# albcab/mfm

Hardware: AMD Instinct MI355X
Metric: MFM train-steps/s x chains (phi-four d=256, 4096 chains per GPU) (higher is better)
Workload: dtype f32

## Files before the change

### include/mfm.h

```cpp
#ifndef MFM_H
#define MFM_H

#include <stddef.h>
#include <stdint.h>

#ifdef __cplusplus
extern "C" {
#endif

typedef struct mfm_ctx mfm_ctx;

enum { MFM_OK = 0, MFM_EINVAL = -1, MFM_EUNSUPPORTED = -2, MFM_ETOOLARGE = -3, MFM_EHIP = -4, MFM_ENOTARGET = -5 };

enum { MFM_PHI4 = 0, MFM_GMM = 1, MFM_LGCP = 2 };
enum { MFM_FLOW_RWMH = 0, MFM_FLOW_IMH = 1 };
enum { MFM_FAMILY_AUTO = 0, MFM_FAMILY_TILE = 1, MFM_FAMILY_WIDE = 2 };
enum { MFM_ACT_RELU = 0, MFM_ACT_TANH = 1, MFM_ACT_ELU = 2, MFM_ACT_GELU = 3, MFM_ACT_SWISH = 4 };

#define MFM_MAX_DEPTH 3
typedef struct mfm_config {
  int32_t dim;
  int32_t fourier_dim;
  int32_t hidden_t[2];
  int32_t hidden_x[2];
// ... 76 lines not shown
int mfm_vf_apply(mfm_ctx* ctx, const float* d_x, const float* d_t, const float* d_tangent, int n,
                 float* d_v, float* d_jvp);
int mfm_ode_transform(mfm_ctx* ctx, int direction, int per_chain_keys, const uint32_t* d_keys, uint32_t key0,
                      uint32_t key1, const float* d_in, int n, float* d_out, float* d_ldj, int32_t* d_nsteps);
int mfm_flow_step(mfm_ctx* ctx, int mode, uint32_t key0, uint32_t key1, double beta,
                  float* d_pos, double* d_logp, float* d_grad,
                  float* d_acceptance_rate, uint8_t* d_is_accepted, float* d_proposed_position, int32_t* d_nsteps);

int mfm_train_iter(mfm_ctx* ctx, int64_t count, int mcmc_per_flow_steps, int flow_mode,
                   uint32_t gen_key0, uint32_t gen_key1, uint32_t train_key0, uint32_t train_key1,
                   double beta, double step_size, float* d_pos, double* d_logp, float* d_grad,
                   float* d_acceptance_rate, int32_t* d_nsteps, double* d_loss, float* d_grads, int apply_update);

int mfm_beta_update(mfm_ctx* ctx, double prev_beta, const double* d_logliks, int n, double alpha, double* h_beta_out);

int mfm_normal_rows(mfm_ctx* ctx, const uint32_t* d_keys, int n, float* d_out);

int mfm_cis_select(mfm_ctx* ctx, uint32_t key0, uint32_t key1, int n_is, const float* d_u0, const float* d_vol0,
                   const float* d_refs, const float* d_xs, const float* d_vols, const double* d_lps, float* d_pos,
                   double* d_logp, float* d_acc_prob, uint8_t* d_is_accepted, float* d_proposed, float* d_weight);

int mfm_stein_disc(mfm_ctx* ctx, const float* d_x, const float* d_grad, int n, double beta, double h_u_v[2]);
int mfm_max_mean_disc(mfm_ctx* ctx, const float* d_x, const float* d_y, int m, double* h_out);

#define MFM_AUTOCORR_LAG_BLOCK 32
#define MFM_AUTOCORR_TIME_BLOCK 256
int mfm_autocorr(mfm_ctx* ctx, const float* d_x, int64_t n, int64_t n_series, int32_t n_lags,
                 float* d_rho      ,
                 float* d_tau, float* d_ess ,
                 double* d_mean, double* d_var );

int mfm_noise_prefetch(mfm_ctx* ctx, int n_slots, const uint32_t* h_keys_gn, const uint32_t* h_keys_step);
int mfm_noise_drop(mfm_ctx* ctx);

int mfm_smc_delta(mfm_ctx* ctx, const double* d_loglik, int n, double target_ess, double max_delta, double* h_delta);
int mfm_smc_weights(mfm_ctx* ctx, const double* d_loglik, int n, double delta, double* d_weights, double* h_lognorm);
int mfm_smc_resample(mfm_ctx* ctx, uint32_t key0, uint32_t key1, const double* d_weights, int n, double* d_scratch,
                     int32_t* d_idx);
#define MFM_RESAMPLE_SYSTEMATIC 0
#define MFM_RESAMPLE_STRATIFIED 1
#define MFM_RESAMPLE_MULTINOMIAL 2
int mfm_smc_resample_scheme(mfm_ctx* ctx, int scheme, uint32_t key0, uint32_t key1, const double* d_weights, int n,
                            double* d_scratch, int32_t* d_idx);
int mfm_gather_rows(mfm_ctx* ctx, const float* d_src, const int32_t* d_idx, int n, int dim, float* d_dst);
int mfm_choice_logw(mfm_ctx* ctx, uint32_t key0, uint32_t key1, const double* d_logw, int n, int m, double* d_scratch,
                    int32_t* d_idx);
int mfm_acc_stats(mfm_ctx* ctx, const float* d_x, int n, double* d_out);

int mfm_get_counters(mfm_ctx* ctx, int64_t h_out[8]);
int mfm_reset_counters(mfm_ctx* ctx);

int mfm_debug_replay(mfm_ctx* ctx, int cap, const float* d_dt, const uint8_t* d_acc, float* d_ratio, float* d_dt_own,
                     double* d_diag);

int mfm_profile(mfm_ctx* ctx, int class_mask);
int mfm_profile_read(mfm_ctx* ctx, double ms_total[8], int64_t launches[8]);

int mfm_pack_index(int k, int n, int KB);
int mfm_pack_index_T(int k, int n, int NB);
int mfm_threefry2x32(uint32_t k0, uint32_t k1, uint32_t c0, uint32_t c1, uint32_t out[2]);

#ifdef __cplusplus
}
#endif
#endif
```

### mfm_amd/_lib.py

```python
import ctypes as C
import os

import numpy as np

from .build import LIB

PHI4, GMM, LGCP = 0, 1, 2
FLOW_RWMH, FLOW_IMH = 0, 1
FAMILY_AUTO, FAMILY_TILE, FAMILY_WIDE = 0, 1, 2
ACTIVATIONS = {"relu": 0, "tanh": 1, "elu": 2, "gelu": 3, "swish": 4}


class MfmError(RuntimeError):
    pass


class Config(C.Structure):
    _fields_ = [
        ("dim", C.c_int32), ("fourier_dim", C.c_int32),
        ("hidden_t", C.c_int32 * 2), ("hidden_x", C.c_int32 * 2), ("hidden_xt", C.c_int32 * 2),
        ("n_chain_local", C.c_int32), ("n_chain_total", C.c_int32), ("chain_offset", C.c_int32),
        ("grad_clip", C.c_float), ("sigma", C.c_float), ("cond_flow", C.c_int32), ("hutch", C.c_int32),
        ("rtol", C.c_double), ("atol", C.c_double), ("mxstep", C.c_int32), ("n_ts", C.c_int32),
        ("learning_rate", C.c_double), ("adam_b1", C.c_double), ("adam_b2", C.c_double), ("adam_eps", C.c_double),
# ... 31 lines not shown
    "mfm_mala_step_keys": (C.c_int, [_P, _P, C.c_double, C.c_double, C.c_int, _P, _P, _P, _P, _P, _P, _P]),
    "mfm_mala_run": (C.c_int, [_P, C.c_int, _U32, _U32, _P, C.c_double, C.c_double, C.c_int, C.c_int32, C.c_int32, _P, _P, _P, _P, _P, _P, _P, _P, _P, _P, _P]),
    "mfm_hmc_step": (C.c_int, [_P, _U32, _U32, C.c_double, C.c_double, C.c_int, _P, _P, _P, _P, _P]),
    "mfm_loglik": (C.c_int, [_P, _P, _P]),
    "mfm_smc_delta": (C.c_int, [_P, _P, C.c_int, C.c_double, C.c_double, C.POINTER(C.c_double)]),
    "mfm_smc_weights": (C.c_int, [_P, _P, C.c_int, C.c_double, _P, C.POINTER(C.c_double)]),
    "mfm_smc_resample": (C.c_int, [_P, _U32, _U32, _P, C.c_int, _P, _P]),
    "mfm_smc_resample_scheme": (C.c_int, [_P, C.c_int, _U32, _U32, _P, C.c_int, _P, _P]),
    "mfm_gather_rows": (C.c_int, [_P, _P, _P, C.c_int, C.c_int, _P]),
    "mfm_acc_stats": (C.c_int, [_P, _P, C.c_int, _P]),
    "mfm_choice_logw": (C.c_int, [_P, _U32, _U32, _P, C.c_int, C.c_int, _P, _P]),
    "mfm_fm_loss_grad": (C.c_int, [_P, _U32, _U32, _P, _P, _P]),
    "mfm_fm_loss": (C.c_int, [_P, _U32, _U32, _P, C.c_int, C.c_int, C.c_int, _P]),
    "mfm_adamw_step": (C.c_int, [_P, _P]),
    "mfm_comm_unique_id": (C.c_int, [_P]),
    "mfm_comm_init": (C.c_int, [_P, C.c_int, C.c_int, _P]),
    "mfm_comm_destroy": (C.c_int, [_P]),
    "mfm_comm_count": (C.c_int, [_P, _P]),
    "mfm_grad_allreduce_begin": (C.c_int, [_P, _P]),
    "mfm_opt_state": (C.c_int, [_P, C.POINTER(C.c_int32), C.POINTER(C.c_float)]),
    "mfm_vf_apply": (C.c_int, [_P, _P, _P, _P, C.c_int, _P, _P]),
    "mfm_ode_transform": (C.c_int, [_P, C.c_int, C.c_int, _P, _U32, _U32, _P, C.c_int, _P, _P, _P]),
    "mfm_flow_step": (C.c_int, [_P, C.c_int, _U32, _U32, C.c_double, _P, _P, _P, _P, _P, _P, _P]),
    "mfm_train_iter": (C.c_int, [_P, C.c_int64, C.c_int, C.c_int, _U32, _U32, _U32, _U32, C.c_double, C.c_double,
                                 _P, _P, _P, _P, _P, _P, _P, C.c_int]),
    "mfm_beta_update": (C.c_int, [_P, C.c_double, _P, C.c_int, C.c_double, C.POINTER(C.c_double)]),
    "mfm_normal_rows": (C.c_int, [_P, _P, C.c_int, _P]),
    "mfm_cis_select": (C.c_int, [_P, _U32, _U32, C.c_int, _P, _P, _P, _P, _P, _P, _P, _P, _P, _P, _P, _P]),
    "mfm_stein_disc": (C.c_int, [_P, _P, _P, C.c_int, C.c_double, C.POINTER(C.c_double)]),
    "mfm_max_mean_disc": (C.c_int, [_P, _P, _P, C.c_int, C.POINTER(C.c_double)]),
    "mfm_autocorr": (C.c_int, [_P, _P, C.c_int64, C.c_int64, C.c_int32, _P, _P, _P, _P, _P]),
    "mfm_noise_prefetch": (C.c_int, [_P, C.c_int, C.POINTER(_U32), C.POINTER(_U32)]),
    "mfm_noise_drop": (C.c_int, [_P]),
    "mfm_get_counters": (C.c_int, [_P, C.POINTER(C.c_int64)]),
    "mfm_reset_counters": (C.c_int, [_P]),
    "mfm_debug_replay": (C.c_int, [_P, C.c_int, _P, _P, _P, _P, _P]),
    "mfm_profile": (C.c_int, [_P, C.c_int]),
    "mfm_profile_read": (C.c_int, [_P, C.POINTER(C.c_double), C.POINTER(C.c_int64)]),
    "mfm_pack_index": (C.c_int, [C.c_int, C.c_int, C.c_int]),
    "mfm_pack_index_T": (C.c_int, [C.c_int, C.c_int, C.c_int]),
    "mfm_threefry2x32": (C.c_int, [_U32, _U32, _U32, _U32, C.POINTER(_U32)]),
}
EXPORTS = tuple(_SIGS)

_lib = None


def load():
    global _lib
    if _lib is None:
        if not os.path.exists(LIB):
            raise MfmError(f"{LIB} not found: build it with `python -m mfm_amd.build` (hipcc, gfx950)")
        import torch
        lib = C.CDLL(os.environ.get("MFM_LIB", LIB))
        for name, (res, args) in _SIGS.items():
            fn = getattr(lib, name)
            fn.restype, fn.argtypes = res, args
        _lib = lib
    return _lib


def _chk(rc):
    if rc != 0:
        raise MfmError(f"libmfm_hip error {rc}: {load().mfm_last_error().decode()}")


# ... 197 lines not shown
        self._p()
        _chk(self.lib.mfm_vf_apply(self.h, _ptr(x, F32), _ptr(t, F32), _ptr(tangent, F32), x.shape[0], _ptr(v, F32), _ptr(jvp, F32)))

    def ode_transform(self, direction, x, out, ldj, keys=None, key=(0, 0), nsteps=None):
        self._p()
        _chk(self.lib.mfm_ode_transform(self.h, direction, 0 if keys is None else 1, _ptr(keys, I32), int(key[0]), int(key[1]),
                                        _ptr(x, F32), x.shape[0], _ptr(out, F32), _ptr(ldj, F32), _ptr(nsteps, I32)))

    def flow_step(self, mode, key, beta, pos, logp, grad, acc=None, is_acc=None, proposed=None, nsteps=None):
        self._p()
        _chk(self.lib.mfm_flow_step(self.h, mode, int(key[0]), int(key[1]), float(beta), _ptr(pos, F32), _ptr(logp, F64), _ptr(grad, F32),
                                    _ptr(acc, F32), _ptr(is_acc, U8), _ptr(proposed, F32), _ptr(nsteps, I32)))

    def train_iter(self, count, mcmc_per_flow_steps, flow_mode, key_gen, key_train, beta, step_size, pos, logp, grad, loss, grads,
                   acc=None, nsteps=None, apply_update=True):
        self._p()
        _chk(self.lib.mfm_train_iter(self.h, int(count), int(mcmc_per_flow_steps), int(flow_mode), int(key_gen[0]), int(key_gen[1]),
                                     int(key_train[0]), int(key_train[1]), float(beta), float(step_size), _ptr(pos, F32), _ptr(logp, F64),
                                     _ptr(grad, F32), _ptr(acc, F32), _ptr(nsteps, I32), _ptr(loss, F64), _ptr(grads, F32),
                                     1 if apply_update else 0))

    def noise_prefetch(self, keys_gn, keys_step):
        kg = np.ascontiguousarray(keys_gn, dtype=np.uint32).reshape(-1, 2)
        ks = np.ascontiguousarray(keys_step, dtype=np.uint32).reshape(-1, 2)
        assert kg.shape == ks.shape
        if kg.shape[0] == 0:
            return False
        rc = self.lib.mfm_noise_prefetch(self.h, kg.shape[0], kg.ctypes.data_as(C.POINTER(_U32)), ks.ctypes.data_as(C.POINTER(_U32)))
        if rc == -2:
            return False
        _chk(rc)
        return True

    def noise_drop(self):
        _chk(self.lib.mfm_noise_drop(self.h))

    COUNTERS = ("mala_chain_steps", "fm_train_samples", "fm_eval_samples", "ode_solves", "dopri_attempts", "field_evals",
                "optimizer_steps", "mala_hbm_bytes")

    def counters(self):
        out = (C.c_int64 * 8)()
        _chk(self.lib.mfm_get_counters(self.h, out))
        return dict(zip(self.COUNTERS, [int(v) for v in out]))

    def reset_counters(self):
        _chk(self.lib.mfm_reset_counters(self.h))

    def debug_replay(self, dt, acc, ratio, dt_own, diag=None):
        cap = dt.shape[-1]
        for t_ in (acc, ratio, dt_own):
            assert t_.shape == dt.shape
        self._replay_keep = (dt, acc, ratio, dt_own, diag)
        _chk(self.lib.mfm_debug_replay(self.h, cap, _ptr(dt, F32), _ptr(acc, U8), _ptr(ratio, F32), _ptr(dt_own, F32), _ptr(diag, F64)))

    PROF_CLASSES = ("mala_step", "fm_fwd_bwd", "wgrad", "adamw", "flow_step", "fm_eval", "reduce", "_")

    def profile(self, enable=True, classes=None):
        mask = 0 if not enable else (-1 if classes is None else sum(1 << self.PROF_CLASSES.index(c) for c in classes))
        _chk(self.lib.mfm_profile(self.h, mask))

    def profile_read(self):
        ms, cnt = (C.c_double * 8)(), (C.c_int64 * 8)()
        _chk(self.lib.mfm_profile_read(self.h, ms, cnt))
        return {n: dict(ms=ms[i], launches=cnt[i]) for i, n in enumerate(self.PROF_CLASSES) if cnt[i]}

    def normal_rows(self, keys, out):
# ... 30 lines not shown
```

### mfm_amd/csrc/api.hip

```cpp
#include "../../include/mfm.h"

#include <cmath>
#include <cstdarg>
#include <cstdio>
#include <cstring>
#include <vector>
#include <dlfcn.h>
#include <mutex>
#include <rccl/rccl.h>

#include "mala.hip"
#include "mala_run.hip"
#include "lgcp.hip"
#include "hmc.hip"
#include "fm.hip"
#include "optim.hip"
#include "wgrad_sk.hip"
#include "noise.hip"
#include "ode.hip"
#include "anneal.hip"
#include "metrics.hip"
#include "diag.hip"
#include "cis.hip"
#include "wide.hip"
// ... 1246 lines not shown
    return fail(MFM_ETOOLARGE, "n_series = %lld / n_lags = %d exceed the launch grid of the autocorrelation kernel", (long long)n_series, n_lags);
  LAUNCHCHK();
  return MFM_OK;
}

extern "C" int mfm_noise_prefetch(mfm_ctx* x, int n_slots, const uint32_t* h_keys_gn, const uint32_t* h_keys_step) { use_ctx(x);
  NEED_TARGET();
  if (!h_keys_gn || !h_keys_step || n_slots <= 0) return fail(MFM_EINVAL, "bad arguments");
  if (x->wide || !x->cfg.cond_flow || !fast::shape_ok(x->net, x->cfg.hutch) || (x->cfg.ode_method != MFM_ODE_DOPRI5 && x->cfg.ode_steps > 0))
    return fail(MFM_EUNSUPPORTED, "the noise prefetch rides in the tail of the shape-specialised flow-step kernel (headline network shape, PhiFour, --hutch)");
  if (!x->noise) x->noise = new NoiseWs();
  NoiseWs* w = x->noise;
  const size_t B = (size_t)x->cfg.n_chain_local, d = (size_t)x->cfg.dim;
  if (n_slots > w->cap) {
    HIPCHK(hipStreamSynchronize(x->stream));
    for (void* p : {(void*)w->mala_n, (void*)w->mala_u, (void*)w->fm_x0, (void*)w->fm_eps, (void*)w->fm_t, (void*)w->d_keys}) if (p) (void)hipFree(p);
    w->cap = n_slots; w->n_valid = 0;
    ALLOC(w->mala_n, (size_t)n_slots * B * d); ALLOC(w->mala_u, (size_t)n_slots * B);
    ALLOC(w->fm_x0, (size_t)n_slots * B * d); ALLOC(w->fm_eps, (size_t)n_slots * B * d); ALLOC(w->fm_t, (size_t)n_slots * B);
    ALLOC(w->d_keys, (size_t)4 * n_slots);
    if (!w->counter) ALLOC(w->counter, 4);
  }
  w->h_keys.assign(h_keys_gn, h_keys_gn + 2 * (size_t)n_slots);
  w->h_keys.insert(w->h_keys.end(), h_keys_step, h_keys_step + 2 * (size_t)n_slots);
  HIPCHK(hipMemcpyAsync(w->d_keys, w->h_keys.data(), w->h_keys.size() * sizeof(uint32_t), hipMemcpyHostToDevice, x->stream));
  w->gn.resize(n_slots); w->st.resize(n_slots);
  for (int j = 0; j < n_slots; ++j) {
    w->gn[j] = Key2{h_keys_gn[2 * j], h_keys_gn[2 * j + 1]};
    w->st[j] = Key2{h_keys_step[2 * j], h_keys_step[2 * j + 1]};
  }
  w->n_armed = n_slots; w->n_valid = 0;
  return MFM_OK;
}
extern "C" int mfm_noise_drop(mfm_ctx* x) { use_ctx(x);
  if (!x) return fail(MFM_EINVAL, "null ctx");
  if (x->noise) { x->noise->n_valid = 0; x->noise->n_armed = 0; }
  return MFM_OK;
}

extern "C" int mfm_smc_delta(mfm_ctx* x, const double* d_ll, int n, double target_ess, double max_delta, double* h_delta) { use_ctx(x);
  if (!x || !d_ll || !h_delta) return fail(MFM_EINVAL, "null argument");
  if (n <= 0) return fail(MFM_EINVAL, "n must be positive");
  hipLaunchKernelGGL(smc_delta_kernel, dim3(1), dim3(SMC_THREADS), 0, x->stream, d_ll, n, target_ess, max_delta, x->beta_out);
  LAUNCHCHK();
  HIPCHK(hipMemcpyAsync(h_delta, x->beta_out, sizeof(double), hipMemcpyDeviceToHost, x->stream));
  HIPCHK(hipStreamSynchronize(x->stream));
  return MFM_OK;
}
extern "C" int mfm_smc_weights(mfm_ctx* x, const double* d_ll, int n, double delta, double* d_weights, double* h_lognorm) { use_ctx(x);
  if (!x || !d_ll || !d_weights) return fail(MFM_EINVAL, "null argument");
  if (n <= 0) return fail(MFM_EINVAL, "n must be positive");
  hipLaunchKernelGGL(smc_weights_kernel, dim3(1), dim3(SMC_THREADS), 0, x->stream, d_ll, n, delta, d_weights, x->beta_out + 1);
  LAUNCHCHK();
  if (h_lognorm) {
    HIPCHK(hipMemcpyAsync(h_lognorm, x->beta_out + 1, sizeof(double), hipMemcpyDeviceToHost, x->stream));
    HIPCHK(hipStreamSynchronize(x->stream));
  }
  return MFM_OK;
}
extern "C" int mfm_smc_resample(mfm_ctx* x, uint32_t k0, uint32_t k1, const double* d_weights, int n, double* d_scratch, int32_t* d_idx) { use_ctx(x);
  if (!x || !d_weights || !d_scratch || !d_idx) return fail(MFM_EINVAL, "null argument");
  if (n <= 0) return fail(MFM_EINVAL, "n must be positive");
  hipLaunchKernelGGL(smc_resample_kernel, dim3(1), dim3(SMC_THREADS), 0, x->stream, Key2{k0, k1}, d_weights, n, d_scratch, d_idx);
  LAUNCHCHK();
  return MFM_OK;
}
// ... 55 lines not shown
```

### mfm_amd/csrc/fm.hip

```cpp
#include <type_traits>
#include "mlp.hip.h"
#include "prng.hip.h"


struct WsLayout {
  int a_ffat, a_t1, a_st, a_cond, a_x1, a_sx, a_j1, a_j2, a_tiles;
  int z_t1, z_t2, z_x1, z_x2, z_gate, z_j1, z_j2, z_out, z_tiles;
};

struct FmMala {
  int on, textbook;
  Key2 key;
  double beta, eps;
  double* logp; float* grad; float* acc_prob;
  const draw_t* pre_n; const double* pre_u;
};

struct FmArgs {
  NetDev net;
  WsLayout ws;
  Key2 key_time, key_ref, key_gauss;
  uint32_t n_total, chain_offset;
  int B;
  int n_valid;
// ... 210 lines not shown
    }
#pragma unroll
    for (int q = 0; q < TPW; ++q) {
      const int nt = wave + MLP_WAVES_FM * q, col = nt * 16 + c;
      const bool live = nt * 16 < n.dp && col < d;
      f32x4 cv = {0.f, 0.f, 0.f, 0.f};
#pragma unroll
      for (int i = 0; i < 4; ++i) {
        tgt[q][i] = 0.f;
        if (live) {
          const double x1v = x1f[q][i], t = tt[i], x0 = a.ref_std * (double)x0d[q][i];
          cv[i] = (float)((double)a.sigma * (double)ned[q][i] + t * x1v + (1.0 - t) * x0);
          tgt[q][i] = (float)(x1v - x0);
          bX[(4 * g + i) * L.ldx + 4 + col] = cv[i];
        }
      }
      if (TRAIN && nt * 16 < n.dp) store_chk(a.acts, a.ws.a_cond + nt, cv);
    }
  } else
#pragma unroll
  for (int q = 0; q < TPW; ++q) {
    const int nt = wave + MLP_WAVES_FM * q, col = nt * 16 + c;
    f32x4 cv = {0.f, 0.f, 0.f, 0.f};
#pragma unroll
    for (int i = 0; i < 4; ++i) {
      tgt[q][i] = 0.f;
      if (nt * 16 < n.dp && col < d) {
        const int row = 4 * g + i;
        const double x1v = x1_at(row, col);
        const double t = tt[i];
        double cnd, tg;
        if (a.cond_flow) {
          const size_t po = (size_t)(b0 + row) * d + col;
          const double x0 = a.ref_std * (double)(a.pre_x0 ? a.pre_x0[po] : (draw_t)normal64(kref[i], (uint32_t)col, (uint32_t)d));
          const double ne = (double)(a.pre_x0 ? a.pre_eps[po] : (draw_t)normal64(a.key_gauss, bglob[i] * (uint32_t)d + (uint32_t)col, a.n_total * (uint32_t)d));
          cnd = (double)a.sigma * ne + t * x1v + (1.0 - t) * x0;
          tg = x1v - x0;
        } else {
          const double x0 = normal64(a.key_ref, bglob[i] * (uint32_t)d + (uint32_t)col, a.n_total * (uint32_t)d);
          const double sds = 1.0 - (1.0 - (double)a.sigma) * t;
          cnd = t * x1v + sds * x0;
          tg = x1v - (1.0 - (double)a.sigma) * x0;
        }
        cv[i] = (float)cnd;
        tgt[q][i] = (float)tg;
        bX[row * L.ldx + 4 + col] = cv[i];
      }
    }
    if (TRAIN && nt * 16 < n.dp) store_chk(a.acts, a.ws.a_cond + nt, cv);
  }
  FM_STAMP(1);
  __syncthreads();
  if (n.T.kind == MFM_TARGET_GMM && (n.T.n_modes <= 16 ? threadIdx.x < 256 : threadIdx.x < 16)) {
    double lp; float gg[8];
    const int row = n.T.n_modes <= 16 ? (int)(threadIdx.x >> 4) : (int)threadIdx.x;
    if (n.T.n_modes <= 16) gmm_eval_lanes16<8>(n.T, bX + row * L.ldx + 4, threadIdx.x & 15, &lp, gg);
    else gmm_eval<8>(n.T, bX + row * L.ldx + 4, &lp, gg);
    if (n.T.n_modes > 16 || (threadIdx.x & 15) == 0)
      for (int j = 0; j < d; ++j) gcs[row * 8 + j] = gg[j];
  }

  FM_STAMP(2);
  auto relu_store = [&](const LayerDesc& ld, float* out, int ldo, int coff, int a_tile) {
    return [&, out, ldo, coff, a_tile](int q, int nt, int m, f32x4 acc, float bias) {
      f32x4 v;
#pragma unroll
      for (int i = 0; i < 4; ++i) {
        v[i] = act_f(acc[i] + bias, n.act);
// ... 695 lines not shown
```

### mfm_amd/csrc/mala.hip

```cpp
#include "mcmc.hip.h"

#define MALA_WAVES 4
#define MALA_MAXD_SMALL 8

struct MalaArgs {
  TargetDev T;
  Key2 key;
  const uint32_t* keys;
  uint32_t n_total, chain_offset;
  int B;
  double beta;
  double eps;
  int textbook;
  float* pos; double* logp; float* grad;
  float* acc_prob; uint8_t* accepted; float* proposed; float* prop_weight;
  const draw_t* pre_n; const double* pre_u;
};

template <int MAXIT, bool BCRT = false>
__device__ __forceinline__ double row_value_grad(const TargetDev& T, double beta, const float* xs, int d, int lane,
                                                 float (&gout)[MAXIT], float* gsm) {
  double acc = 0.0;
  if (T.kind == MFM_TARGET_PHI4) {
#pragma unroll
// ... 106 lines not shown
  double lp0[NCH], u0[NCH];
#pragma unroll
  for (int c = 0; c < NCH; ++c) {
    const size_t row = (size_t)b[c] * d;
    th1[c] = 0.0; k_int[c] = Key2{0, 0}; k_rmh[c] = Key2{0, 0};
    lp0[c] = a.logp[b[c]];
    u0[c] = a.pre_u ? a.pre_u[b[c]] : 0.0;
    if (lane == 0) { xs[c][-1] = 0.f; xs[c][d] = 0.f; }
    if (!a.pre_n) {
      const Key2 kb = mcmc_chain_key(a.key, a.keys, a.n_total, a.chain_offset, b[c]);
      k_int[c] = mcmc_step_key(kb, MCMC_K_INT);
      k_rmh[c] = mcmc_step_key(kb, MCMC_K_RMH);
    } else {
#pragma unroll
      for (int it = 0; it < MAXIT; ++it) { const int j = lane + 64 * it; nz[c][it] = j < d ? a.pre_n[row + j] : (draw_t)0; }
    }
#pragma unroll
    for (int it = 0; it < MAXIT; ++it) {
      const int j = lane + 64 * it;
      if (j < d) { x[c][it] = a.pos[row + j]; g[c][it] = a.grad[row + j]; }
    }
  }
  FM_STAMP(10);
  __builtin_amdgcn_sched_barrier(0);
  after_loads();
  __builtin_amdgcn_sched_barrier(0);
  FM_STAMP(11);
#pragma unroll
  for (int c = 0; c < NCH; ++c) {
#pragma unroll
    for (int it = 0; it < MAXIT; ++it) {
      const int j = lane + 64 * it;
      if (j < d) {
        const double n = a.pre_n ? (double)nz[c][it] : (double)(draw_t)normal64(k_int[c], (uint32_t)j, (uint32_t)d);
        xn[c][it] = mala_propose<false>(x[c][it], g[c][it], n, a.eps, s2e, th1[c]);
        xs[c][j] = xn[c][it];
      }
    }
  }
  __builtin_amdgcn_fence(__ATOMIC_RELEASE, "workgroup");
  __builtin_amdgcn_wave_barrier();
  __builtin_amdgcn_fence(__ATOMIC_ACQUIRE, "workgroup");

  FM_STAMP(12);
  float gn[NCH][MAXIT];
  double lpn[NCH], th2[NCH];
#pragma unroll
  for (int c = 0; c < NCH; ++c) {
    lpn[c] = row_value_grad<MAXIT, BCRT>(a.T, a.beta, xs[c], d, lane, gn[c], gsm[c]);
    th2[c] = 0.0;
#pragma unroll
    for (int it = 0; it < MAXIT; ++it) {
      const int j = lane + 64 * it;
      if (j < d) mala_back<false>(x[c][it], xn[c][it], gn[c][it], a.eps, th2[c]);
    }
  }
  FM_STAMP(13);
#pragma unroll
  for (int c = 0; c < NCH; ++c) { th1[c] = wave_sum(th1[c]); th2[c] = wave_sum(th2[c]); }
  FM_STAMP(14);
#pragma unroll
  for (int c = 0; c < NCH; ++c) {
    const size_t row = (size_t)b[c] * d;
    const double p = mala_accept_p<false>(lp0[c], lpn[c], th1[c], th2[c], a.eps, a.textbook);
    const double u = a.pre_u ? u0[c] : uniform01(k_rmh[c], 0, 1);
    const bool acc = u < p;
#pragma unroll
// ... 55 lines not shown
```

### mfm_amd/csrc/mala_run.hip

```cpp

struct MalaRunArgs {
  MalaArgs m;
  int key_mode;
  int n_steps, thin;
  int32_t* n_acc;
  double* acc_sum;
  float* traj_pos;
  double* traj_logp;
};

__device__ __attribute__((noinline)) double run_normal64(Key2 key, uint32_t idx, uint32_t size) { return normal64(key, idx, size); }
__device__ __attribute__((noinline)) double run_uniform01(Key2 key) { return uniform01(key, 0, 1); }
__device__ __attribute__((noinline)) double run_exp(double v) { return exp(v); }
struct RunExp { __device__ __forceinline__ double operator()(double v) const { return run_exp(v); } };

template <int MAXIT, bool BCRT = false>
__global__ __launch_bounds__(MALA_WAVES * 64) void mala_run_kernel(MalaRunArgs r) {
  extern __shared__ __attribute__((aligned(16))) float smem[];
  const MalaArgs& a = r.m;
  const int d = a.T.dim, lane = threadIdx.x & 63, wave = threadIdx.x >> 6;
  const int rowlen = d + 2;
  const int b = blockIdx.x * MALA_WAVES + wave;
  if (b >= a.B) return;
  float* const xs = smem + wave * rowlen + 1;
  float* const gsm = smem + MALA_WAVES * rowlen + wave * MALA_MAXD_SMALL;
  const size_t row = (size_t)b * d;
  const size_t B = (size_t)a.B;

  float x[MAXIT], g[MAXIT], xn[MAXIT];
  double lp = a.logp[b];
#pragma unroll
  for (int it = 0; it < MAXIT; ++it) {
    const int j = lane + 64 * it;
    x[it] = 0.f; g[it] = 0.f; xn[it] = 0.f;
    if (j < d) { x[it] = a.pos[row + j]; g[it] = a.grad[row + j]; }
  }
  if (lane == 0) { xs[-1] = 0.f; xs[d] = 0.f; }
  const Key2 kc = r.key_mode ? Key2{a.keys[2 * b], a.keys[2 * b + 1]} : Key2{0, 0};
  const double s2e = mala_s2e(a.eps);
  int n_acc = 0;
  double acc_sum = 0.0, p_last = 0.0, pw_last = 0.0;
  bool acc_last = false;

  for (int s = 0; s < r.n_steps; ++s) {
    const Key2 kb = mcmc_run_key(r.key_mode, a.key, kc, (uint32_t)r.n_steps, (uint32_t)s, a.n_total, a.chain_offset + (uint32_t)b);
    const Key2 k_int = mcmc_step_key(kb, MCMC_K_INT), k_rmh = mcmc_step_key(kb, MCMC_K_RMH);
    double th1 = 0.0;
#pragma unroll
    for (int it = 0; it < MAXIT; ++it) {
      const int j = lane + 64 * it;
      if (j < d) {
        const double n = (double)(draw_t)run_normal64(k_int, (uint32_t)j, (uint32_t)d);
        xn[it] = mala_propose<false>(x[it], g[it], n, a.eps, s2e, th1);
        xs[j] = xn[it];
      }
    }
    __builtin_amdgcn_fence(__ATOMIC_RELEASE, "workgroup");
    __builtin_amdgcn_wave_barrier();
    __builtin_amdgcn_fence(__ATOMIC_ACQUIRE, "workgroup");

    float gn[MAXIT];
#pragma unroll
    for (int it = 0; it < MAXIT; ++it) gn[it] = 0.f;
    const double lpn = row_value_grad<MAXIT, BCRT>(a.T, a.beta, xs, d, lane, gn, gsm);
    double th2 = 0.0;
#pragma unroll
    for (int it = 0; it < MAXIT; ++it) {
      const int j = lane + 64 * it;
      if (j < d) mala_back<false>(x[it], xn[it], gn[it], a.eps, th2);
    }
    th1 = wave_sum(th1); th2 = wave_sum(th2);
    const double p = mala_accept_p<false>(lp, lpn, th1, th2, a.eps, a.textbook, RunExp());
    const double u = run_uniform01(k_rmh);
    const bool acc = u < p;
    const double lpn0 = __shfl(lpn, 0, 64);
#pragma unroll
    for (int it = 0; it < MAXIT; ++it) {
      x[it] = acc ? xn[it] : x[it];
      g[it] = acc ? gn[it] : g[it];
    }
    lp = acc ? lpn0 : lp;
    n_acc += acc ? 1 : 0;
    acc_sum += p;
    if (s == r.n_steps - 1) {
      p_last = p; acc_last = acc;
// ... 57 lines not shown
```

### mfm_amd/csrc/noise.hip

```cpp
#pragma once
#include "common.hip.h"
#include "prng.hip.h"

struct NoiseArgs {
  const uint32_t* gn; const uint32_t* st;
  int n_slots; uint32_t n_total, chain_offset; int B, d;
  draw_t* mala_n; double* mala_u;
  draw_t* fm_x0; draw_t* fm_eps; float* fm_t;
  int* counter; int n_items, groups;
  int skip_mala0;
};

__device__ __forceinline__ void noise_row(const NoiseArgs& a, int slot, int b, int lane) {
  const uint32_t bg = a.chain_offset + (uint32_t)b, d = (uint32_t)a.d;
  const size_t row = ((size_t)slot * a.B + b) * a.d, one = (size_t)slot * a.B + b;
  if (!(a.skip_mala0 && slot == 0)) {
    const Key2 kg{a.gn[2 * slot], a.gn[2 * slot + 1]};
    const Key2 kb = split_at(kg, a.n_total, bg);
    const Key2 k_int = split_at(kb, 2, 0), k_rmh = split_at(kb, 2, 1);
    for (int j = lane; j < a.d; j += 64) a.mala_n[row + j] = (draw_t)normal64(k_int, (uint32_t)j, d);
    if (lane == 0) a.mala_u[one] = uniform01(k_rmh, 0, 1);
  }
  {
    const Key2 ks{a.st[2 * slot], a.st[2 * slot + 1]};
    const Key2 key_time = split_at(ks, 4, 0), key_ref = split_at(ks, 4, 1), key_gauss = split_at(ks, 4, 2);
    const Key2 kref = split_at(key_ref, a.n_total, bg);
    for (int j = lane; j < a.d; j += 64) {
      a.fm_x0[row + j] = (draw_t)normal64(kref, (uint32_t)j, d);
      a.fm_eps[row + j] = (draw_t)normal64(key_gauss, bg * d + (uint32_t)j, a.n_total * d);
    }
    if (lane == 0) a.fm_t[one] = (float)uniform01(key_time, bg, a.n_total);
  }
}

__device__ __noinline__ void noise_tail(const NoiseArgs& a, volatile int* slot_word) {
  const int lane = threadIdx.x & 63, wave = threadIdx.x >> 6;
  for (;;) {
    __syncthreads();
    if (threadIdx.x == 0) *slot_word = atomicAdd(a.counter, 1);
    __syncthreads();
    const int item = *slot_word;
    if (item >= a.n_items) break;
    const int slot = item / a.groups, b = (item - slot * a.groups) * 8 + wave;
    if (b < a.B) noise_row(a, slot, b, lane);
  }
}
```

### mfm_amd/csrc/ode.hip

```cpp
#include "dopri5.hip.h"
#include "mlp.hip.h"
#include "prng.hip.h"

struct PadWs { float* Wp; float* WpT; float* bias; float* img[6]; size_t rows; int D; };
struct OdeWs { float* noise; size_t rows; f32x4* fast_scr; size_t fast_wgs; PadWs pad; };
static thread_local const PadWs* t_pad = nullptr;
#define ODE_FAST_MAX_WGS 1024
#define ODE_FAST_SCR_F4 (5 * 8 * 3 * 64)
static int flow_live_rows(int n_chains) {
  if (g_sw.flow_live == 16 || g_sw.flow_live == 8 || g_sw.flow_live == 4 || g_sw.flow_live == 2) return g_sw.flow_live;
  int live = 16;
  while (live > 2 && n_chains / (live / 2) <= 256) live /= 2;
  return live;
}

static int ode_ws_alloc(const NetDev& n, const mfm_config& c, OdeWs& w) {
  w.rows = (size_t)(c.max_eval_samples > c.n_chain_local ? c.max_eval_samples : c.n_chain_local);
  if (hipMalloc((void**)&w.noise, 3 * w.rows * n.d * sizeof(float)) != hipSuccess) return -4;
  const size_t t_all = w.rows / 16, t_chain = (size_t)c.n_chain_local / 16;
  w.fast_wgs = t_all < ODE_FAST_MAX_WGS ? t_all : ODE_FAST_MAX_WGS;
  const size_t t_flow = (size_t)c.n_chain_local / flow_live_rows(c.n_chain_local);
  if (w.fast_wgs < t_flow) w.fast_wgs = t_flow;
  memset(&w.pad, 0, sizeof w.pad);
  if (c.hutch && n.nT == 2 && n.nX == 2 && n.nJ == 2 && !net_ragged(n) && n.T.kind == MFM_TARGET_PHI4 && n.act == MFM_ACT_RELU && n.F == 128 && n.ht1 == 128 && n.ht2 == 128 && n.hx1 == 128 &&
// ... 713 lines not shown
            dn_n[i] = 1.f;
          } else {
            ell_n[i] = l1;
#pragma unroll
            for (int q = 0; q < TPW; ++q) { y[q][i] = xin[q][i]; k[0][q][i] = k[6][q][i]; }
            kl0_n[i] = kl[6][i];
          }
          t_n[i] = tn;
        }
        dt_n[i] = active ? ndt : dti;
        na_n[i] = active ? na4[i] + 1.f : na4[i];
        any |= (dn_n[i] == 0.f && na_n[i] < (float)max_attempts && dt_n[i] > 0.f);
      }
      T.rs_put(RS_T, t_n); T.rs_put(RS_DT, dt_n); T.rs_put(RS_ELL, ell_n); T.rs_put(RS_KL + 0, kl0_n);
      T.rs_put(RS_NATT, na_n); T.rs_put(RS_DONE, dn_n);
      if (!__syncthreads_or(any ? 1 : 0)) break;
      phase = 2;
    }
  }
  {
    const f32x4 ell4 = T.rs_get(RS_ELL), na4 = T.rs_get(RS_NATT);
#pragma unroll
    for (int i = 0; i < 4; ++i) { ell[i] = ell4[i]; natt[i] = (int)na4[i]; }
  }
}

__global__ __launch_bounds__(256) void probe_kernel(int mode, const uint32_t* keys, Key2 key, uint32_t n_total, uint32_t chain_offset,
                                                   int sub, int n, int d, float* out) {
  const int lane = threadIdx.x & 63, b = blockIdx.x * 4 + (threadIdx.x >> 6);
  if (b >= n) return;
  Key2 k = key;
  if (mode == 0) k = Key2{keys[2 * b], keys[2 * b + 1]};
  else if (mode == 2) k = split_at(split_at(key, n_total, chain_offset + (uint32_t)b), 4, (uint32_t)sub);
  for (int j = lane; j < d; j += 64) out[(size_t)b * d + j] = (float)normal64(k, (uint32_t)j, (uint32_t)d);
}
static void launch_probe(int mode, const uint32_t* keys, Key2 key, uint32_t n_total, uint32_t chain_offset, int sub, int n, int d,
                         float* out, hipStream_t stream) {
  hipLaunchKernelGGL(probe_kernel, dim3((n + 3) / 4), dim3(256), 0, stream, mode, keys, key, n_total, chain_offset, sub, n, d, out);
}

template <int TPW, int NW>
__device__ __forceinline__ void fill_probe(OdeTile<TPW, NW>& T, const float* z, int b0, bool hutch) {
  const NetDev& N = *T.n;
#pragma unroll
  for (int q = 0; q < TPW; ++q) {
    const int col = (T.wave + NW * q) * 16 + T.c;
    if (col < N.dp) {
#pragma unroll
      for (int i = 0; i < 4; ++i)
        T.bZ()[(4 * T.g + i) * T.L.ldx + 4 + col] = (hutch && col < N.d) ? z[(size_t)(b0 + 4 * T.g + i) * N.d + col] : 0.f;
    }
  }
}

template <int TPW, int NW>
__device__ __forceinline__ void tile_init(OdeTile<TPW, NW>& T, const NetDev* n, float* lds, bool hutch) {
  T.n = n; T.L = ode_lds_layout(*n, NW); T.lds = lds;
  T.lane = threadIdx.x & 63; T.wave = __builtin_amdgcn_readfirstlane(threadIdx.x >> 6); T.g = T.lane >> 4; T.c = T.lane & 15;
  T.hutch = hutch; T.exact = false; T.sign = 1;
  for (int i = threadIdx.x; i < T.L.total; i += (NW * 64)) lds[i] = 0.f;
#pragma unroll
  for (int i = 0; i < 4; ++i) {
    T.tz1[0][i] = 0.f; T.tz1[1][i] = 0.f;
#pragma unroll
    for (int q = 0; q < TPW; ++q) T.gate[q][i] = 0.f;
  }
  __syncthreads();
// ... 417 lines not shown
```

### mfm_amd/csrc/prng.hip.h

```cpp
#pragma once
#include "common.hip.h"

struct Key2 { uint32_t k0, k1; };

__host__ __device__ __forceinline__ uint32_t rotl32(uint32_t x, int r) { return (x << r) | (x >> (32 - r)); }

__host__ __device__ __forceinline__ void threefry2x32(Key2 key, uint32_t c0, uint32_t c1, uint32_t& o0, uint32_t& o1) {
  const uint32_t ks0 = key.k0, ks1 = key.k1, ks2 = key.k0 ^ key.k1 ^ 0x1BD11BDAu;
  uint32_t x0 = c0 + ks0, x1 = c1 + ks1;
#define TF_R(r) x0 += x1; x1 = rotl32(x1, r); x1 ^= x0;
  TF_R(13) TF_R(15) TF_R(26) TF_R(6)   x0 += ks1; x1 += ks2 + 1u;
  TF_R(17) TF_R(29) TF_R(16) TF_R(24)  x0 += ks2; x1 += ks0 + 2u;
  TF_R(13) TF_R(15) TF_R(26) TF_R(6)   x0 += ks0; x1 += ks1 + 3u;
  TF_R(17) TF_R(29) TF_R(16) TF_R(24)  x0 += ks1; x1 += ks2 + 4u;
  TF_R(13) TF_R(15) TF_R(26) TF_R(6)   x0 += ks2; x1 += ks0 + 5u;
#undef TF_R
  o0 = x0; o1 = x1;
}

__host__ __device__ __forceinline__ Key2 split_at(Key2 key, uint32_t num, uint32_t idx) {
  Key2 r;
  uint32_t w[2];
#pragma unroll
  for (int q = 0; q < 2; ++q) {
    uint32_t m = 2u * idx + q;
    bool lo = m < num;
    uint32_t c0 = lo ? m : m - num;
    uint32_t y0, y1;
    threefry2x32(key, c0, c0 + num, y0, y1);
    w[q] = lo ? y0 : y1;
  }
  r.k0 = w[0]; r.k1 = w[1];
  return r;
}

__host__ __device__ __forceinline__ uint64_t random_bits64(Key2 key, uint32_t idx, uint32_t size) {
  uint32_t y0, y1;
  threefry2x32(key, idx, idx + size, y0, y1);
  return ((uint64_t)y0 << 32) | (uint64_t)y1;
}

__device__ __forceinline__ double bits_to_unit(uint64_t bits) {
  return __longlong_as_double((long long)((bits >> 12) | 0x3FF0000000000000ULL)) - 1.0;
}

__device__ __forceinline__ double uniform01(Key2 key, uint32_t idx, uint32_t size) {
  return fmax(0.0, bits_to_unit(random_bits64(key, idx, size)));
}

__device__ __forceinline__ double normal64(Key2 key, uint32_t idx, uint32_t size) {
  const double lo = -0.99999999999999988897769753748;
  const double span = 1.0 - lo;
  double u = bits_to_unit(random_bits64(key, idx, size));
  u = __dadd_rn(__dmul_rn(u, span), lo);
  u = fmax(lo, u);
#ifdef MFM_EXP_FAKE_NORMAL
  return u;
#else
  return 1.4142135623730951 * erfinv(u);
#endif
}
```

Measured before the change: 6.001 million.

## Add fast float normal sampler with guarded fallback to exact double erfinv

Replaces the double-precision erfinv-based Gaussian draw with a polynomial approximation in double (custom log plus degree-24 polynomial). It checks whether the float-rounded result is stable under a small perturbation and falls back to the exact double path only when any lane in the wavefront fails that check. The noise prefetch kernel also hoists per-slot key splitting out of the per-row loop and uses nontemporal stores. A debug entry point is added to compare fast and reference normals. The intent is to cut the cost of the double erfinv that dominates random draws, at the price of wave-level divergence when a fallback is needed.

```diff
diff --git a/include/mfm.h b/include/mfm.h
--- a/include/mfm.h
+++ b/include/mfm.h
@@ -132,6 +132,8 @@
 
 int mfm_noise_prefetch(mfm_ctx* ctx, int n_slots, const uint32_t* h_keys_gn, const uint32_t* h_keys_step);
 int mfm_noise_drop(mfm_ctx* ctx);
+int mfm_debug_normals(mfm_ctx* ctx, uint32_t k0, uint32_t k1, uint32_t size, uint32_t first, const uint64_t* d_raw, int64_t n,
+                      float* d_out_fast, float* d_out_ref, uint8_t* d_out_slow_mask);
 
 int mfm_smc_delta(mfm_ctx* ctx, const double* d_loglik, int n, double target_ess, double max_delta, double* h_delta);
 int mfm_smc_weights(mfm_ctx* ctx, const double* d_loglik, int n, double delta, double* d_weights, double* h_lognorm);
diff --git a/mfm_amd/_lib.py b/mfm_amd/_lib.py
--- a/mfm_amd/_lib.py
+++ b/mfm_amd/_lib.py
@@ -87,6 +87,7 @@
     "mfm_autocorr": (C.c_int, [_P, _P, C.c_int64, C.c_int64, C.c_int32, _P, _P, _P, _P, _P]),
     "mfm_noise_prefetch": (C.c_int, [_P, C.c_int, C.POINTER(_U32), C.POINTER(_U32)]),
     "mfm_noise_drop": (C.c_int, [_P]),
+    "mfm_debug_normals": (C.c_int, [_P, _U32, _U32, _U32, _U32, _P, C.c_int64, _P, _P, _P]),
     "mfm_get_counters": (C.c_int, [_P, C.POINTER(C.c_int64)]),
     "mfm_reset_counters": (C.c_int, [_P]),
     "mfm_debug_replay": (C.c_int, [_P, C.c_int, _P, _P, _P, _P, _P]),
@@ -350,6 +351,12 @@
         _chk(rc)
         return True
 
+    def debug_normals(self, out_fast, out_ref, out_slow=None, key=(0, 0), size=0, first=0, raw=None):
+        n = out_fast.numel()
+        assert out_ref.numel() == n and (out_slow is None or out_slow.numel() == n) and (raw is None or raw.numel() == n)
+        _chk(self.lib.mfm_debug_normals(self.h, int(key[0]), int(key[1]), int(size), int(first), _ptr(raw, "int64"), n,
+                                        _ptr(out_fast, F32), _ptr(out_ref, F32), _ptr(out_slow, U8)))
+
     def noise_drop(self):
         _chk(self.lib.mfm_noise_drop(self.h))
 
diff --git a/mfm_amd/csrc/api.hip b/mfm_amd/csrc/api.hip
--- a/mfm_amd/csrc/api.hip
+++ b/mfm_amd/csrc/api.hip
@@ -1302,6 +1302,14 @@
   w->n_armed = n_slots; w->n_valid = 0;
   return MFM_OK;
 }
+extern "C" int mfm_debug_normals(mfm_ctx* x, uint32_t k0, uint32_t k1, uint32_t size, uint32_t first, const uint64_t* d_raw, int64_t n,
+                                 float* d_out_fast, float* d_out_ref, uint8_t* d_out_slow_mask) { use_ctx(x);
+  if (!x || !d_out_fast || !d_out_ref) return fail(MFM_EINVAL, "null argument");
+  if (n <= 0 || n > ((int64_t)1 << 31)) return fail(MFM_EINVAL, "n must be in 1 .. 2^31");
+  launch_debug_normals(Key2{k0, k1}, size, first, d_raw, (long long)n, d_out_fast, d_out_ref, d_out_slow_mask, x->stream);
+  LAUNCHCHK();
+  return MFM_OK;
+}
 extern "C" int mfm_noise_drop(mfm_ctx* x) { use_ctx(x);
   if (!x) return fail(MFM_EINVAL, "null ctx");
   if (x->noise) { x->noise->n_valid = 0; x->noise->n_armed = 0; }
diff --git a/mfm_amd/csrc/fm.hip b/mfm_amd/csrc/fm.hip
--- a/mfm_amd/csrc/fm.hip
+++ b/mfm_amd/csrc/fm.hip
@@ -266,8 +266,8 @@
         double cnd, tg;
         if (a.cond_flow) {
           const size_t po = (size_t)(b0 + row) * d + col;
-          const double x0 = a.ref_std * (double)(a.pre_x0 ? a.pre_x0[po] : (draw_t)normal64(kref[i], (uint32_t)col, (uint32_t)d));
-          const double ne = (double)(a.pre_x0 ? a.pre_eps[po] : (draw_t)normal64(a.key_gauss, bglob[i] * (uint32_t)d + (uint32_t)col, a.n_total * (uint32_t)d));
+          const double x0 = a.ref_std * (double)(a.pre_x0 ? a.pre_x0[po] : (draw_t)normal32(kref[i], (uint32_t)col, (uint32_t)d));
+          const double ne = (double)(a.pre_x0 ? a.pre_eps[po] : (draw_t)normal32(a.key_gauss, bglob[i] * (uint32_t)d + (uint32_t)col, a.n_total * (uint32_t)d));
           cnd = (double)a.sigma * ne + t * x1v + (1.0 - t) * x0;
           tg = x1v - x0;
         } else {
diff --git a/mfm_amd/csrc/mala.hip b/mfm_amd/csrc/mala.hip
--- a/mfm_amd/csrc/mala.hip
+++ b/mfm_amd/csrc/mala.hip
@@ -162,7 +162,7 @@
     for (int it = 0; it < MAXIT; ++it) {
       const int j = lane + 64 * it;
       if (j < d) {
-        const double n = a.pre_n ? (double)nz[c][it] : (double)(draw_t)normal64(k_int[c], (uint32_t)j, (uint32_t)d);
+        const double n = a.pre_n ? (double)nz[c][it] : (double)(draw_t)normal32(k_int[c], (uint32_t)j, (uint32_t)d);
         xn[c][it] = mala_propose<false>(x[c][it], g[c][it], n, a.eps, s2e, th1[c]);
         xs[c][j] = xn[c][it];
       }
diff --git a/mfm_amd/csrc/mala_run.hip b/mfm_amd/csrc/mala_run.hip
--- a/mfm_amd/csrc/mala_run.hip
+++ b/mfm_amd/csrc/mala_run.hip
@@ -9,7 +9,7 @@
   double* traj_logp;
 };
 
-__device__ __attribute__((noinline)) double run_normal64(Key2 key, uint32_t idx, uint32_t size) { return normal64(key, idx, size); }
+__device__ __attribute__((noinline)) float run_normal32(Key2 key, uint32_t idx, uint32_t size) { return normal32(key, idx, size); }
 __device__ __attribute__((noinline)) double run_uniform01(Key2 key) { return uniform01(key, 0, 1); }
 __device__ __attribute__((noinline)) double run_exp(double v) { return exp(v); }
 struct RunExp { __device__ __forceinline__ double operator()(double v) const { return run_exp(v); } };
@@ -50,7 +50,7 @@
     for (int it = 0; it < MAXIT; ++it) {
       const int j = lane + 64 * it;
       if (j < d) {
-        const double n = (double)(draw_t)run_normal64(k_int, (uint32_t)j, (uint32_t)d);
+        const double n = (double)(draw_t)run_normal32(k_int, (uint32_t)j, (uint32_t)d);
         xn[it] = mala_propose<false>(x[it], g[it], n, a.eps, s2e, th1);
         xs[j] = xn[it];
       }
diff --git a/mfm_amd/csrc/noise.hip b/mfm_amd/csrc/noise.hip
--- a/mfm_amd/csrc/noise.hip
+++ b/mfm_amd/csrc/noise.hip
@@ -11,37 +11,59 @@
   int skip_mala0;
 };
 
-__device__ __forceinline__ void noise_row(const NoiseArgs& a, int slot, int b, int lane) {
+struct NoiseSlotKeys { Key2 kg, key_time, key_ref, key_gauss; };
+
+__device__ __forceinline__ NoiseSlotKeys noise_slot_keys(const NoiseArgs& a, int slot) {
+  const Key2 ks{a.st[2 * slot], a.st[2 * slot + 1]};
+  return NoiseSlotKeys{Key2{a.gn[2 * slot], a.gn[2 * slot + 1]}, split_at(ks, 4, 0), split_at(ks, 4, 1), split_at(ks, 4, 2)};
+}
+
+__device__ __forceinline__ void noise_row(const NoiseArgs& a, const NoiseSlotKeys& K, int slot, int b, int lane) {
   const uint32_t bg = a.chain_offset + (uint32_t)b, d = (uint32_t)a.d;
   const size_t row = ((size_t)slot * a.B + b) * a.d, one = (size_t)slot * a.B + b;
   if (!(a.skip_mala0 && slot == 0)) {
-    const Key2 kg{a.gn[2 * slot], a.gn[2 * slot + 1]};
-    const Key2 kb = split_at(kg, a.n_total, bg);
+    const Key2 kb = split_at(K.kg, a.n_total, bg);
     const Key2 k_int = split_at(kb, 2, 0), k_rmh = split_at(kb, 2, 1);
-    for (int j = lane; j < a.d; j += 64) a.mala_n[row + j] = (draw_t)normal64(k_int, (uint32_t)j, d);
+    for (int j = lane; j < a.d; j += 64) __builtin_nontemporal_store((draw_t)normal32(k_int, (uint32_t)j, d), &a.mala_n[row + j]);
     if (lane == 0) a.mala_u[one] = uniform01(k_rmh, 0, 1);
   }
   {
-    const Key2 ks{a.st[2 * slot], a.st[2 * slot + 1]};
-    const Key2 key_time = split_at(ks, 4, 0), key_ref = split_at(ks, 4, 1), key_gauss = split_at(ks, 4, 2);
-    const Key2 kref = split_at(key_ref, a.n_total, bg);
+    const Key2 kref = split_at(K.key_ref, a.n_total, bg);
     for (int j = lane; j < a.d; j += 64) {
-      a.fm_x0[row + j] = (draw_t)normal64(kref, (uint32_t)j, d);
-      a.fm_eps[row + j] = (draw_t)normal64(key_gauss, bg * d + (uint32_t)j, a.n_total * d);
+      __builtin_nontemporal_store((draw_t)normal32(kref, (uint32_t)j, d), &a.fm_x0[row + j]);
+      __builtin_nontemporal_store((draw_t)normal32(K.key_gauss, bg * d + (uint32_t)j, a.n_total * d), &a.fm_eps[row + j]);
     }
-    if (lane == 0) a.fm_t[one] = (float)uniform01(key_time, bg, a.n_total);
+    if (lane == 0) a.fm_t[one] = (float)uniform01(K.key_time, bg, a.n_total);
   }
 }
 
 __device__ __noinline__ void noise_tail(const NoiseArgs& a, volatile int* slot_word) {
-  const int lane = threadIdx.x & 63, wave = threadIdx.x >> 6;
+  const int lane = threadIdx.x & 63, wave = __builtin_amdgcn_readfirstlane(threadIdx.x >> 6);
+  int cur = -1;
+  NoiseSlotKeys K{};
   for (;;) {
     __syncthreads();
     if (threadIdx.x == 0) *slot_word = atomicAdd(a.counter, 1);
     __syncthreads();
-    const int item = *slot_word;
+    const int item = __builtin_amdgcn_readfirstlane(*slot_word);
     if (item >= a.n_items) break;
     const int slot = item / a.groups, b = (item - slot * a.groups) * 8 + wave;
-    if (b < a.B) noise_row(a, slot, b, lane);
+    if (slot != cur) { K = noise_slot_keys(a, slot); cur = slot; }
+    if (b < a.B) noise_row(a, K, slot, b, lane);
   }
 }
+
+__global__ __launch_bounds__(256) void debug_normals_kernel(Key2 key, uint32_t size, uint32_t first, const uint64_t* raw, long long n,
+                                                           float* out_fast, float* out_ref, uint8_t* out_slow) {
+  const long long i = (long long)blockIdx.x * 256 + threadIdx.x;
+  if (i >= n) return;
+  const uint64_t bits = raw ? raw[i] : random_bits64(key, first + (uint32_t)i, size);
+  bool slow;
+  out_fast[i] = normal32_bits(bits, &slow);
+  out_ref[i] = (float)normal64_bits(bits);
+  if (out_slow) out_slow[i] = slow ? 1 : 0;
+}
+static void launch_debug_normals(Key2 key, uint32_t size, uint32_t first, const uint64_t* raw, long long n, float* out_fast, float* out_ref,
+                                 uint8_t* out_slow, hipStream_t stream) {
+  hipLaunchKernelGGL(debug_normals_kernel, dim3((unsigned)((n + 255) / 256)), dim3(256), 0, stream, key, size, first, raw, n, out_fast, out_ref, out_slow);
+}
diff --git a/mfm_amd/csrc/ode.hip b/mfm_amd/csrc/ode.hip
--- a/mfm_amd/csrc/ode.hip
+++ b/mfm_amd/csrc/ode.hip
@@ -769,7 +769,7 @@
   Key2 k = key;
   if (mode == 0) k = Key2{keys[2 * b], keys[2 * b + 1]};
   else if (mode == 2) k = split_at(split_at(key, n_total, chain_offset + (uint32_t)b), 4, (uint32_t)sub);
-  for (int j = lane; j < d; j += 64) out[(size_t)b * d + j] = (float)normal64(k, (uint32_t)j, (uint32_t)d);
+  for (int j = lane; j < d; j += 64) out[(size_t)b * d + j] = normal32(k, (uint32_t)j, (uint32_t)d);
 }
 static void launch_probe(int mode, const uint32_t* keys, Key2 key, uint32_t n_total, uint32_t chain_offset, int sub, int n, int d,
                          float* out, hipStream_t stream) {
diff --git a/mfm_amd/csrc/prng.hip.h b/mfm_amd/csrc/prng.hip.h
--- a/mfm_amd/csrc/prng.hip.h
+++ b/mfm_amd/csrc/prng.hip.h
@@ -48,10 +48,10 @@
   return fmax(0.0, bits_to_unit(random_bits64(key, idx, size)));
 }
 
-__device__ __forceinline__ double normal64(Key2 key, uint32_t idx, uint32_t size) {
+__device__ __forceinline__ double normal64_bits(uint64_t bits) {
   const double lo = -0.99999999999999988897769753748;
   const double span = 1.0 - lo;
-  double u = bits_to_unit(random_bits64(key, idx, size));
+  double u = bits_to_unit(bits);
   u = __dadd_rn(__dmul_rn(u, span), lo);
   u = fmax(lo, u);
 #ifdef MFM_EXP_FAKE_NORMAL
@@ -60,3 +60,68 @@
   return 1.4142135623730951 * erfinv(u);
 #endif
 }
+__device__ __forceinline__ double normal64(Key2 key, uint32_t idx, uint32_t size) { return normal64_bits(random_bits64(key, idx, size)); }
+
+#define NORMAL32_W0 8.0
+#define NORMAL32_G 0x1p-38
+#define NORMAL32_FAST_BOUND 0x1p-45
+
+__host__ __device__ __forceinline__ double normal32_u(uint64_t bits) {
+#pragma clang fp contract(off)
+  const double lo = -0.99999999999999988897769753748;
+  const double span = 1.0 - lo;
+  double u = __builtin_bit_cast(double, (bits >> 12) | 0x3FF0000000000000ULL) - 1.0;
+#if defined(__HIP_DEVICE_COMPILE__)
+  u = __dadd_rn(__dmul_rn(u, span), lo);
+#else
+  u = u * span;
+  u = u + lo;
+#endif
+  return fmax(lo, u);
+}
+
+__host__ __device__ __forceinline__ double normal32_log(double t) {
+#pragma clang fp contract(off)
+  uint64_t ix = __builtin_bit_cast(uint64_t, t) + 0x00095F6200000000ULL;
+  const double e = (double)((int)(ix >> 52) - 1023);
+  const double m = __builtin_bit_cast(double, (ix & 0x000FFFFFFFFFFFFFULL) + 0x3FE6A09E00000000ULL);
+  const double s = (m - 1.0) / (m + 1.0), s2 = s * s;
+  double q = 1.0 / 19.0;
+  q = fma(q, s2, 1.0 / 17.0); q = fma(q, s2, 1.0 / 15.0); q = fma(q, s2, 1.0 / 13.0); q = fma(q, s2, 1.0 / 11.0);
+  q = fma(q, s2, 1.0 / 9.0);  q = fma(q, s2, 1.0 / 7.0);  q = fma(q, s2, 1.0 / 5.0);  q = fma(q, s2, 1.0 / 3.0);
+  const double s_2 = s + s;
+  return fma(e, 0.6931471805599453, fma(s_2 * s2, q, s_2));
+}
+
+__host__ __device__ __forceinline__ double normal32_fast(double u, double& w) {
+#pragma clang fp contract(off)
+  w = -normal32_log((1.0 - u) * (1.0 + u));
+  const double x = fma(w, 2.0 / 8.25, -1.0);
+  double p = -0x1.12492546d9adap-28;
+  p = fma(p, x, -0x1.3deceb1d97d06p-24); p = fma(p, x, 0x1.7b68791e94ce8p-23);  p = fma(p, x, 0x1.b4d273921eea7p-22);
+  p = fma(p, x, -0x1.817c3b8bf4a69p-20); p = fma(p, x, 0x1.175d79be4c90ap-23);  p = fma(p, x, 0x1.374f9b75a9724p-18);
+  p = fma(p, x, -0x1.055c1a3286c2ap-17); p = fma(p, x, 0x1.3294fe3d09620p-25);  p = fma(p, x, 0x1.a42f872caa935p-16);
+  p = fma(p, x, -0x1.b70e2c869218cp-15); p = fma(p, x, 0x1.6e4fb7a24fe44p-16);  p = fma(p, x, 0x1.26bc1742c376cp-13);
+  p = fma(p, x, -0x1.875482849abf7p-12); p = fma(p, x, 0x1.281535a379d28p-12);  p = fma(p, x, 0x1.869590a4931cfp-11);
+  p = fma(p, x, -0x1.568412776ac42p-9);  p = fma(p, x, 0x1.81fdc98b56ac3p-9);   p = fma(p, x, 0x1.9514e84ab1160p-9);
+  p = fma(p, x, -0x1.27633828a0025p-6);  p = fma(p, x, 0x1.0341edfa72930p-5);   p = fma(p, x, -0x1.51f33e3b4d580p-7);
+  p = fma(p, x, -0x1.fbdaaffa5ff60p-4);  p = fma(p, x, 0x1.de74402cc22b8p-1);   p = fma(p, x, 0x1.e32035fcfe7a8p+0);
+  return (1.4142135623730951 * u) * p;
+}
+
+__host__ __device__ __forceinline__ bool normal32_try(double u, float& z) {
+#pragma clang fp contract(off)
+  double w;
+  const double f = normal32_fast(u, w);
+  z = (float)f;
+  return (w < NORMAL32_W0) & (u != 0.0) & ((float)(f * (1.0 + NORMAL32_G)) == (float)(f * (1.0 - NORMAL32_G)));
+}
+
+__device__ __forceinline__ float normal32_bits(uint64_t bits, bool* slow = nullptr) {
+  float z;
+  const bool ok = normal32_try(normal32_u(bits), z);
+  if (slow) *slow = !ok;
+  if (__any(!ok)) z = (float)normal64_bits(bits);
+  return z;
+}
+__device__ __forceinline__ float normal32(Key2 key, uint32_t idx, uint32_t size) { return normal32_bits(random_bits64(key, idx, size)); }
```

New measurement: 5.996 million, median of 3. About the same (-0.1%).
